# igd-geo/schwarzwald

Measured on AMD Instinct MI355X. Metric: Mpoints/s end-to-end tile (Morton+sort+sample), higher is better.
Workload: dtype u64 keys / f64 positions

## Files before the change

### schwarzwald_amd/csrc/swz_mdblock.hip

```cpp
#include <algorithm>
#include <cmath>
#include <cstdio>
#include <cstdlib>

#include "swz_md.h"
#include "swz_scan.h"

namespace swz {

#ifndef SB_MINW
#define SB_MINW 6
#endif
constexpr int SB_THREADS = 256;
constexpr int SB_K = 4;
constexpr int SB_PEND = 63;
constexpr uint32_t SB_CNT_SAT = 128;
static_assert(SB_CNT_SAT + SB_PEND <= 255u, "a point's neighbour count must not carry into the next point's byte");
static_assert(SB_CNT_SAT > (uint32_t)SB_K, "a saturated count must still read as 'more than the list holds'");
constexpr int SB_PMAX = 12;
constexpr uint32_t SB_NC = 64;
constexpr uint32_t SB_CTR_STRIDE = 32;
constexpr uint32_t SB_NONE = 0xFFFFFFFFu;
enum : uint32_t { SB_U = 0, SB_A = 1, SB_R = 2 };
enum : uint32_t { SB_ABORT_NONE = 0, SB_ABORT_CAPACITY = 1, SB_ABORT_TIMEOUT = 2 };
enum : uint32_t { SBW_ABORT = 0, SBW_MAX_OWN = 1, SBW_MAX_HALO = 2, SBW_ITER = 3, SBW_BLOCKS = 4, SBW_WAITS = 5, SBW_RESEARCH = 6, SBW_STEPS = 7,
                  SBW_T0 = 8 , SBW_COUNT = 16 };
#ifdef SWZ_SB_STATS
#define SB_T(i) do { if (tid == 0) { const uint64_t now_ = wall_clock64(); tacc[i] += (uint32_t)(now_ - tlast); tlast = now_; } } while (0)
#else
#define SB_T(i) do { } while (0)
#endif
enum : uint32_t { SBM_SN = 0, SBM_B = 1, SBM_FIRST = 2, SBM_NOWN = 3, SBM_ABORT = 4, SBM_COUNT = 8 };

struct SbArgs {
  const uint64_t* akey;
  uint32_t m;
  const uint2* gtab;
  uint32_t* st2;
  uint8_t* taken;
  const uint32_t* aidx;
  const uint32_t* perm;
  const double* xyz;
  float f_lo, f_hi;
  uint32_t i_lo, i_hi;
  double sq_spacing;
  uint32_t cell_bits;
  uint32_t cl;
  uint32_t ns;
  uint32_t* ctr;
  uint32_t own_cap, halo_cap;
  uint64_t timeout_ticks;
};

__device__ __forceinline__ uint32_t sb_expand3(uint32_t v) {
  v = (v | (v << 16)) & 0x030000FFu;
  v = (v | (v << 8)) & 0x0300F00Fu;
  v = (v | (v << 4)) & 0x030C30C3u;
  v = (v | (v << 2)) & 0x09249249u;
  return v;
}
__device__ __forceinline__ uint32_t sb_load_word(const uint32_t* p) { return __hip_atomic_load(p, __ATOMIC_RELAXED, __HIP_MEMORY_SCOPE_AGENT); }
__device__ __forceinline__ uint32_t sb_lds_state(const uint8_t* st, uint32_t q) {
  return __hip_atomic_load(st + q, __ATOMIC_RELAXED, __HIP_MEMORY_SCOPE_WORKGROUP);
}
__device__ __forceinline__ void sb_lds_set(uint8_t* st, uint32_t q, uint32_t v) {
  __hip_atomic_store(st + q, (uint8_t)v, __ATOMIC_RELAXED, __HIP_MEMORY_SCOPE_WORKGROUP);
}
__device__ __forceinline__ uint64_t sb_pack(uint32_t x, uint32_t y, uint32_t z) { return (uint64_t)x | ((uint64_t)y << 21) | ((uint64_t)z << 42); }
__device__ __forceinline__ void sb_unpack(uint64_t p, uint32_t& x, uint32_t& y, uint32_t& z) {
  const uint32_t lo = (uint32_t)p, hi = (uint32_t)(p >> 32);
  x = lo & 0x1FFFFFu;
  y = ((lo >> 21) | (hi << 11)) & 0x1FFFFFu;
  z = hi >> 10;
}
constexpr uint32_t SB_CELL_NONE = 0xFFFu;

__device__ __forceinline__ bool sb_exact_near(const SbArgs& a, uint32_t gp, uint32_t gq) {
  const uint32_t sp = a.aidx ? a.aidx[gp] : gp, sq = a.aidx ? a.aidx[gq] : gq;
  const double* u = a.xyz + (size_t)a.perm[sp] * 3;
  const double* v = a.xyz + (size_t)a.perm[sq] * 3;
  return sq_dist(u[0], u[1], u[2], v[0], v[1], v[2]) < a.sq_spacing;
}

struct SbLds {
  uint64_t* pts;
  uint32_t* cse;
  uint32_t* occ;
  uint32_t* soff;
  uint32_t* sfirst;
  uint32_t* pub;
  uint32_t* misc;
  uint32_t* scan;
  uint16_t* nbr;
  uint8_t* st;
  uint32_t* cnt4;
  uint32_t* pend;
};
__host__ __device__ inline size_t sb_lds_bytes(uint32_t own_cap, uint32_t halo_cap) {
  const size_t tot = (size_t)own_cap + halo_cap;
  size_t b = tot * 8;
  b += 1024 * 4 + 128 * 4 + 224 * 4 + 224 * 4;
  b += (((size_t)own_cap / 16 + 5) & ~(size_t)1) * 4 + SBM_COUNT * 4 + 8 * 4;
  b += std::max((size_t)own_cap * SB_K, tot) * 2;
  b += ((tot + 3) & ~(size_t)3) + own_cap + 4 * (SB_PEND + 1) * 4;
  return (b + 15) & ~(size_t)15;
}
__device__ __forceinline__ SbLds sb_carve(unsigned char* smem, uint32_t own_cap, uint32_t halo_cap) {
  const uint32_t tot = own_cap + halo_cap;
  SbLds l;
  l.pts = reinterpret_cast<uint64_t*>(smem);
  l.cse = reinterpret_cast<uint32_t*>(l.pts + tot);
  l.occ = l.cse + 1024;
  l.soff = l.occ + 128;
  l.sfirst = l.soff + 224;
  l.pub = l.sfirst + 224;
  l.misc = l.pub + ((own_cap / 16 + 5u) & ~1u);
  l.scan = l.misc + SBM_COUNT;
  l.nbr = reinterpret_cast<uint16_t*>(l.scan + 8);
  l.st = reinterpret_cast<uint8_t*>(l.nbr + max(own_cap * (uint32_t)SB_K, tot));
  l.cnt4 = reinterpret_cast<uint32_t*>(l.st + ((tot + 3u) & ~3u));
  l.pend = l.cnt4 + own_cap / 4u;
  return l;
}

struct SbBlock {
  uint32_t first;
  uint32_t n_own;
  uint32_t bx8, by8, bz8;
};
__device__ __forceinline__ uint32_t sb_region_cell(const SbArgs& a, const SbBlock& k, uint32_t x, uint32_t y, uint32_t z) {
  const uint32_t cmask = (1u << a.cl) - 1u;
  const uint32_t ix = ((x >> a.cell_bits) & cmask) - k.bx8 + 1u, iy = ((y >> a.cell_bits) & cmask) - k.by8 + 1u, iz = ((z >> a.cell_bits) & cmask) - k.bz8 + 1u;
  return (ix < 10u && iy < 10u && iz < 10u) ? (ix | (iy << 4) | (iz << 8)) : SB_CELL_NONE;
}
__device__ __forceinline__ uint32_t sb_cell_index(uint32_t c) { return (c & 15u) + 10u * ((c >> 4) & 15u) + 100u * (c >> 8); }
template <bool WIDE>
__device__ __forceinline__ uint64_t sb_make_point(const SbArgs& a, const SbBlock& k, uint32_t x, uint32_t y, uint32_t z, uint32_t* cell) {
  const uint32_t c = sb_region_cell(a, k, x, y, z);
  *cell = c;
  if (WIDE) return sb_pack(x, y, z);
  const uint32_t nmask = (1u << (a.cell_bits + a.cl)) - 1u;
  const uint32_t xr = (x & nmask) - ((k.bx8 - 1u) << a.cell_bits), yr = (y & nmask) - ((k.by8 - 1u) << a.cell_bits),
                 zr = (z & nmask) - ((k.bz8 - 1u) << a.cell_bits);
  return (uint64_t)((xr & 0xFFFFu) | (yr << 16)) | ((uint64_t)((zr & 0xFFFFu) | (c << 16)) << 32);
}
__device__ __forceinline__ uint32_t sb_halo_slot(const SbLds& l, uint32_t j) {
  uint32_t lo = 0;
#pragma unroll
  for (uint32_t step = 128u; step; step >>= 1)
    if (lo + step <= 216u && l.soff[lo + step] <= j) lo += step;
  return lo;
}
__device__ __forceinline__ uint32_t sb_active_index(const SbLds& l, const SbBlock& k, uint32_t q) {
  if (q < k.n_own) return k.first + q;
  const uint32_t slot = sb_halo_slot(l, q);
  return l.sfirst[slot] + (q - l.soff[slot]);
}

__device__ __forceinline__ uint32_t sb_earlier_mask(uint32_t ix, uint32_t iy, uint32_t iz) {
  const uint32_t lx = ix - 1u, ly = iy - 1u, lz = iz - 1u;
  const int mx = 3 * (int)__builtin_ctz(lx | 8u) + 2, my = 3 * (int)__builtin_ctz(ly | 8u) + 1, mz = 3 * (int)__builtin_ctz(lz | 8u);
  const int px = 3 * (int)__builtin_ctz(~lx) + 2, py = 3 * (int)__builtin_ctz(~ly) + 1, pz = 3 * (int)__builtin_ctz(~lz);
  uint32_t m = 0x361Bu;
  m |= (mx > py ? 1u : 0u) << 15;
  m |= (my > px ? 1u : 0u) << 11;
  m |= (mx > pz ? 1u : 0u) << 21;
  m |= (mz > px ? 1u : 0u) << 5;
  m |= (my > pz ? 1u : 0u) << 19;
  m |= (mz > py ? 1u : 0u) << 7;
  m |= (max(mx, my) > pz ? 1u : 0u) << 18;
  m |= (max(mx, mz) > py ? 1u : 0u) << 6;
  m |= (max(my, mz) > px ? 1u : 0u) << 2;
  m |= (mx > max(py, pz) ? 1u : 0u) << 24;
  m |= (my > max(px, pz) ? 1u : 0u) << 20;
  m |= (mz > max(px, py) ? 1u : 0u) << 8;
  const uint32_t hx = (ix == 1u ? 1u : 0u) | (ix == 8u ? 4u : 0u);
  const uint32_t hy = (iy == 1u ? 7u : 0u) | (iy == 8u ? 7u << 6 : 0u);
  const uint32_t hz = (iz == 1u ? 0x1FFu : 0u) | (iz == 8u ? 0x1FFu << 18 : 0u);
  return m | hx * 0x1249249u | hy * 0x40201u | hz;
}

struct SbOwn {
  uint32_t ux, uy, uz;
  float fx, fy, fz;
  uint32_t corner;
  uint32_t mask;
};
template <bool WIDE>
__device__ __forceinline__ SbOwn sb_own_point(const SbArgs& a, const SbLds& l, const SbBlock& k, uint32_t j) {
  SbOwn p;
  const uint64_t me = l.pts[j];
  uint32_t cell;
  if (WIDE) {
    sb_unpack(me, p.ux, p.uy, p.uz);
    cell = sb_region_cell(a, k, p.ux, p.uy, p.uz);
  } else {
    const uint32_t lo = (uint32_t)me, hi = (uint32_t)(me >> 32);
    p.ux = lo & 0xFFFFu;
    p.uy = lo >> 16;
    p.uz = hi & 0xFFFFu;
    cell = hi >> 16;
  }
  p.fx = (float)p.ux;
  p.fy = (float)p.uy;
  p.fz = (float)p.uz;
  const uint32_t ix = cell & 15u, iy = (cell >> 4) & 15u, iz = cell >> 8;
  uint32_t mask = 0;
#pragma unroll
  for (int i = 0; i < 9; ++i) {
    const uint32_t row = l.occ[(iz + (uint32_t)(i / 3) - 1u) * 10u + (iy + (uint32_t)(i % 3) - 1u)];
    mask |= ((row >> (ix - 1u)) & 7u) << (3 * i);
  }
  mask &= sb_earlier_mask(ix, iy, iz);
  if (!WIDE && mask) {
    const uint32_t cs = 1u << a.cell_bits;
    const int ox = (int)(p.ux & (cs - 1u)), oy = (int)(p.uy & (cs - 1u)), oz = (int)(p.uz & (cs - 1u));
    const uint32_t gx[3] = {(uint32_t)__mul24(ox, ox), 0u, (uint32_t)__mul24((int)cs - ox, (int)cs - ox)};
    const uint32_t gy[3] = {(uint32_t)__mul24(oy, oy), 0u, (uint32_t)__mul24((int)cs - oy, (int)cs - oy)};
    const uint32_t gz[3] = {(uint32_t)__mul24(oz, oz), 0u, (uint32_t)__mul24((int)cs - oz, (int)cs - oz)};
    uint32_t reach = 0;
#pragma unroll 1
    for (int zi = 0; zi < 3; ++zi) {
      const uint32_t gzz = zi == 0 ? gz[0] : (zi == 1 ? 0u : gz[2]);
      uint32_t r9 = 0;
#pragma unroll
      for (int b = 0; b < 9; ++b)
        if (gx[b % 3] + gy[b / 3] + gzz < a.i_hi) r9 |= 1u << b;
      reach |= r9 << (9 * zi);
    }
    mask &= reach;
  }
  p.mask = mask;
  p.corner = (ix - 1u) + 10u * (iy - 1u) + 100u * (iz - 1u);
  return p;
}
template <bool WIDE>
__device__ __forceinline__ void sb_compare(const SbArgs& a, const SbOwn& p, uint64_t o, bool& sure, bool& maybe) {
  if (WIDE) {
    uint32_t vx, vy, vz;
    sb_unpack(o, vx, vy, vz);
    const float ddx = p.fx - (float)vx, ddy = p.fy - (float)vy, ddz = p.fz - (float)vz;
    const float d2 = ddx * ddx + ddy * ddy + ddz * ddz;
    sure = d2 < a.f_lo;
    maybe = d2 < a.f_hi;
  } else {
    const uint32_t lo = (uint32_t)o, hi = (uint32_t)(o >> 32);
    const int ddx = (int)p.ux - (int)(lo & 0xFFFFu), ddy = (int)p.uy - (int)(lo >> 16), ddz = (int)p.uz - (int)(hi & 0xFFFFu);
    const uint32_t d2 = (uint32_t)(__mul24(ddx, ddx) + __mul24(ddy, ddy) + __mul24(ddz, ddz));
    sure = d2 < a.i_lo;
    maybe = d2 < a.i_hi;
  }
}
__device__ __forceinline__ uint32_t sb_cell_offset(uint32_t b) {
  const uint32_t dz = (b * 57u) >> 9, rem = b - 9u * dz, dy = (rem * 11u) >> 5, dx = rem - 3u * dy;
  return dx + 10u * dy + 100u * dz;
}

template <bool WIDE, typename F>
__device__ __forceinline__ void sb_visit(const SbArgs& a, const SbLds& l, const SbBlock& k, uint32_t j, F f) {
  const SbOwn p = sb_own_point<WIDE>(a, l, k, j);
  uint32_t mask = p.mask;
  uint32_t q = 0, e = 0;
  for (;;) {
    if (q >= e) {
      if (!mask) break;
      const uint32_t b = (uint32_t)__ffs((int)mask) - 1u;
      mask &= mask - 1u;
      const uint32_t e2 = l.cse[p.corner + sb_cell_offset(b)];
      q = e2 & 0xFFFFu;
      e = e2 >> 16;
      if (q < k.n_own) e = min(e, j);
      if (q >= e) continue;
    }
    bool sure, maybe;
    sb_compare<WIDE>(a, p, l.pts[q], sure, maybe);
    if (maybe) {
      if (sure || sb_exact_near(a, k.first + j, sb_active_index(l, k, q))) {
        if (!f(q)) return;
      }
    }
    ++q;
  }
}

template <bool WIDE>
__device__ __forceinline__ void sb_search(const SbArgs& a, const SbLds& l, const SbBlock& k, uint32_t j, bool active, uint16_t* mine,
                                          uint32_t* pend, uint32_t* cnt_out, uint32_t* steps) {
  const SbOwn p = sb_own_point<WIDE>(a, l, k, active ? j : 0u);
  uint32_t mask = active ? p.mask : 0u;
  uint32_t q = 0, e = 0, cnt = 0;
  uint32_t ne2 = l.cse[mask ? p.corner + sb_cell_offset((uint32_t)__ffs((int)mask) - 1u) : 0u];
  while (__ballot(active)) {
    ++*steps;
    const bool need = active && q >= e;
    const bool fetch = need && mask != 0u;
    const uint32_t s2 = ne2 & 0xFFFFu, t2 = ne2 >> 16;
    const uint32_t t3 = s2 < k.n_own ? min(t2, j) : t2;
    mask = fetch ? (mask & (mask - 1u)) : mask;
    q = fetch ? s2 : q;
    e = fetch ? t3 : e;
    active = active && !(need && !fetch);
    if (__ballot(fetch)) {
      const uint32_t nxt = l.cse[(fetch && mask) ? p.corner + sb_cell_offset((uint32_t)__ffs((int)mask) - 1u) : 0u];
      ne2 = fetch ? nxt : ne2;
    }
    const bool valid = active && q < e;
    bool sure, maybe;
    sb_compare<WIDE>(a, p, l.pts[valid ? q : 0u], sure, maybe);
    maybe = maybe && valid;
    if (__ballot(maybe)) {
      const bool band = maybe && !sure;
      bool near = maybe && sure;
      if (__ballot(band)) {
        if (band) {
          const uint32_t slot = atomicAdd(&pend[SB_PEND], 1u);
          if (slot < (uint32_t)SB_PEND) pend[slot] = (j << 16) | q;
          else near = sb_exact_near(a, k.first + j, sb_active_index(l, k, q));
        }
      }
      if (near && cnt < (uint32_t)SB_K) mine[cnt] = (uint16_t)q;
      cnt += near ? 1u : 0u;
    }
    q += valid ? 1u : 0u;
  }
  *cnt_out = cnt;
}

__device__ __forceinline__ uint32_t sb_state_of(const SbArgs& a, const SbLds& l, const SbBlock& k, uint32_t q, bool poll) {
  uint32_t s = sb_lds_state(l.st, q);
  if (poll && s == SB_U && q >= k.n_own) {
    const uint32_t gi = sb_active_index(l, k, q);
    s = (sb_load_word(a.st2 + (gi >> 4)) >> ((gi & 15u) * 2u)) & 3u;
    if (s != SB_U) sb_lds_set(l.st, q, s);
  }
  return s;
}

template <bool WIDE>
__global__ __launch_bounds__(SB_THREADS, SB_MINW) void sb_block_kernel(SbArgs a) {
  extern __shared__ __align__(16) unsigned char sb_smem[];
  const SbLds l = sb_carve(sb_smem, a.own_cap, a.halo_cap);
  const uint32_t tid = threadIdx.x, lane = tid & 63u, wave = tid >> 6;
  const uint32_t nb_per_node = 1u << (3u * (a.cl - 3u));
  const uint32_t gmax = 1u << (a.cl - 1u);
  const uint64_t gran_per_node = 1ull << (3u * (a.cl - 1u));
  uint32_t* words = a.ctr + SB_NC * SB_CTR_STRIDE;
  uint32_t kc = (blockIdx.x & 7u) + 8u * ((blockIdx.x >> 3) % (SB_NC / 8u));
  uint32_t tried = 0;
  uint32_t my_blocks = 0, my_iters = 0, my_waits = 0, my_research = 0, my_steps = 0;
  uint16_t* rc = l.nbr;
#ifdef SWZ_SB_STATS
  uint32_t tacc[8] = {0, 0, 0, 0, 0, 0, 0, 0};
  uint64_t tlast = wall_clock64();
#endif
  if (tid == 0) l.misc[SBM_ABORT] = 0;

  for (;;) {
    if (tid == 0) {
      uint32_t sn = SB_NONE, b = 0;
      if (l.misc[SBM_ABORT] == 0 && sb_load_word(words + SBW_ABORT) == SB_ABORT_NONE) {
        while (tried < SB_NC) {
          const uint32_t nodes_k = a.ns > kc ? (a.ns - kc + SB_NC - 1u) / SB_NC : 0u;
          if (nodes_k) {
            const uint32_t t = __hip_atomic_fetch_add(a.ctr + kc * SB_CTR_STRIDE, 1u, __ATOMIC_RELAXED, __HIP_MEMORY_SCOPE_AGENT);
            if ((uint64_t)t < (uint64_t)nodes_k * nb_per_node) {
              sn = (t % nodes_k) * SB_NC + kc;
              b = t / nodes_k;
              break;
            }
          }
          kc = (kc + 1u) % SB_NC;
          ++tried;
        }
      }
      l.misc[SBM_SN] = sn;
      l.misc[SBM_B] = b;
      l.misc[SBM_FIRST] = SB_NONE;
      l.misc[SBM_NOWN] = 0;
    }
    if (tid < 128u) l.occ[tid] = 0u;
    __syncthreads();
    SB_T(0);
    const uint32_t sn = l.misc[SBM_SN], b = l.misc[SBM_B];
    if (sn == SB_NONE) break;

    const uint32_t bx = contract_bits_by_3_u32(b >> 2), by = contract_bits_by_3_u32(b >> 1), bz = contract_bits_by_3_u32(b);
    const uint2* gt = a.gtab + (uint64_t)sn * gran_per_node;
    uint32_t own_cnt = 0, halo_cnt = 0, run_first = 0;
    if (tid < 216u) {
      const uint32_t rx = tid % 6u, ry = (tid / 6u) % 6u, rz = tid / 36u;
      const int gx = (int)(bx * 4u + rx) - 1, gy = (int)(by * 4u + ry) - 1, gz = (int)(bz * 4u + rz) - 1;
      const bool inner = rx - 1u < 4u && ry - 1u < 4u && rz - 1u < 4u;
      if (gx >= 0 && gy >= 0 && gz >= 0 && gx < (int)gmax && gy < (int)gmax && gz < (int)gmax) {
        const uint32_t code = (sb_expand3((uint32_t)gx) << 2) | (sb_expand3((uint32_t)gy) << 1) | sb_expand3((uint32_t)gz);
        if (inner || code < (b << 6)) {
          const uint2 e = gt[code];
          if (e.y) {
            run_first = e.x;
            if (inner) own_cnt = e.y - e.x; else halo_cnt = e.y - e.x;
          }
        }
      }
      if (own_cnt) {
        atomicMin(&l.misc[SBM_FIRST], run_first);
        atomicAdd(&l.misc[SBM_NOWN], own_cnt);
      }
      l.sfirst[tid] = run_first;
    }
    uint32_t n_halo = 0;
    const uint32_t halo_off = block_excl_sum<SB_THREADS>(min(halo_cnt, 0xFFFFFu), l.scan, n_halo);
    SbBlock k;
    k.n_own = l.misc[SBM_NOWN];
    k.first = l.misc[SBM_FIRST];
    k.bx8 = bx * 8u;
    k.by8 = by * 8u;
    k.bz8 = bz * 8u;
    const uint32_t n_own = k.n_own;
    if (n_own == 0) {
      __syncthreads();
      continue;
    }
    const uint32_t total = n_own + n_halo;
    if (n_own > a.own_cap || n_halo > a.halo_cap) {
      if (tid == 0) {
        __hip_atomic_fetch_max(words + SBW_MAX_OWN, n_own, __ATOMIC_RELAXED, __HIP_MEMORY_SCOPE_AGENT);
        __hip_atomic_fetch_max(words + SBW_MAX_HALO, n_halo, __ATOMIC_RELAXED, __HIP_MEMORY_SCOPE_AGENT);
        __hip_atomic_fetch_max(words + SBW_ABORT, (uint32_t)SB_ABORT_CAPACITY, __ATOMIC_RELAXED, __HIP_MEMORY_SCOPE_AGENT);
      }
      break;
    }
    if (tid < 216u) l.soff[tid] = n_own + halo_off;
    if (tid == 216u) l.soff[216] = total;
    const uint32_t w0 = k.first >> 4;
    const uint32_t nw = ((k.first + n_own - 1u) >> 4) - w0 + 1u;
    for (uint32_t w = tid; w < nw; w += SB_THREADS) l.pub[w] = 0u;
    __syncthreads();
    SB_T(1);

#pragma unroll 1
    for (uint32_t half = 0; half < (uint32_t)SB_PMAX; half += 3u) {
      if (half * SB_THREADS >= total) break;
      uint32_t gi[3];
#pragma unroll
      for (int p = 0; p < 3; ++p) {
        const uint32_t j = tid + (half + (uint32_t)p) * SB_THREADS;
        gi[p] = SB_NONE;
        if (j < n_own) {
          gi[p] = k.first + j;
        } else if (j < total) {
          const uint32_t lo = sb_halo_slot(l, j);
          gi[p] = l.sfirst[lo] + (j - l.soff[lo]);
        }
      }
      uint64_t key[3];
      uint32_t sw[3];
#pragma unroll
      for (int p = 0; p < 3; ++p) {
        const uint32_t j = tid + (half + (uint32_t)p) * SB_THREADS;
        key[p] = 0;
        sw[p] = 0;
        if (gi[p] != SB_NONE) {
          key[p] = a.akey[gi[p]];
          if (j >= n_own) sw[p] = sb_load_word(a.st2 + (gi[p] >> 4));
        }
      }
#pragma unroll
      for (int p = 0; p < 3; ++p) {
        const uint32_t j = tid + (half + (uint32_t)p) * SB_THREADS;
        if (gi[p] == SB_NONE) continue;
        uint32_t x, y, z, cell;
        key_coords_u32(key[p], x, y, z);
        l.pts[j] = sb_make_point<WIDE>(a, k, x, y, z, &cell);
        rc[j] = (uint16_t)cell;
        l.st[j] = (uint8_t)((sw[p] >> ((gi[p] & 15u) * 2u)) & 3u);
      }
    }
    __syncthreads();
    SB_T(2);
    for (uint32_t j = tid; j < total; j += SB_THREADS) {
      const uint32_t r = rc[j];
      if (r == SB_CELL_NONE) continue;
      uint16_t* e = reinterpret_cast<uint16_t*>(l.cse + sb_cell_index(r));
      if (j == 0 || rc[j - 1] != r) {
        e[0] = (uint16_t)j;
        atomicOr(&l.occ[(r >> 8) * 10u + ((r >> 4) & 15u)], 1u << (r & 15u));
      }
      if (j + 1 == total || rc[j + 1] != r) e[1] = (uint16_t)(j + 1);
    }
    __syncthreads();
    SB_T(3);

    const uint32_t wa = wave * nw / 4u, wb = (wave + 1u) * nw / 4u;
    const uint32_t ja = max(k.first, (w0 + wa) << 4) - k.first;
    const uint32_t jb = wa < wb ? min(k.first + n_own, (w0 + wb) << 4) - k.first : ja;
    uint32_t* pend = l.pend + wave * (uint32_t)(SB_PEND + 1);
    uint8_t* cnt1 = reinterpret_cast<uint8_t*>(l.cnt4);
    if (lane == 0) pend[SB_PEND] = 0u;
    for (uint32_t base = ja; base < jb; base += 64u) {
      const uint32_t j = base + lane;
      const bool have = j < jb;
      uint32_t cnt = 0;
      sb_search<WIDE>(a, l, k, j, have, l.nbr + (size_t)(have ? j : 0u) * SB_K, pend, &cnt, &my_steps);
      if (have) cnt1[j] = (uint8_t)min(cnt, SB_CNT_SAT);
    }
    {
      const uint32_t np = min(pend[SB_PEND], (uint32_t)SB_PEND);
      for (uint32_t i = lane; i < np; i += 64u) {
        const uint32_t j = pend[i] >> 16, q = pend[i] & 0xFFFFu;
        if (!sb_exact_near(a, k.first + j, sb_active_index(l, k, q))) continue;
        const uint32_t slot = (atomicAdd(&l.cnt4[j >> 2], 1u << (8u * (j & 3u))) >> (8u * (j & 3u))) & 0xFFu;
        if (slot < (uint32_t)SB_K) l.nbr[(size_t)j * SB_K + slot] = (uint16_t)q;
      }
    }
    for (uint32_t base = ja; base < jb; base += 64u) {
      const uint32_t j = base + lane;
      if (j >= jb) continue;
      const uint32_t cnt = cnt1[j];
      uint32_t dec = SB_U;
      if (cnt == 0u) {
        dec = SB_A;
      } else {
        static_assert(SB_K == 4, "four two-byte entries = one eight-byte load");
        uint64_t* slot = reinterpret_cast<uint64_t*>(l.nbr + (size_t)j * SB_K);
        const uint64_t n4 = *slot;
        const uint32_t c4 = min(cnt, (uint32_t)SB_K);
        uint32_t st[SB_K];
#pragma unroll
        for (int i = 0; i < SB_K; ++i) st[i] = (uint32_t)i < c4 ? sb_lds_state(l.st, (uint32_t)(n4 >> (16 * i)) & 0xFFFFu) : (uint32_t)SB_R;
        uint64_t kept = 0;
        uint32_t nk = 0;
        bool any_a = false;
#pragma unroll
        for (int i = 0; i < SB_K; ++i) {
          any_a |= st[i] == SB_A;
          if (st[i] == SB_U) {
            kept |= ((n4 >> (16 * i)) & 0xFFFFull) << (16u * nk);
            ++nk;
          }
        }
        if (any_a) {
          dec = SB_R;
        } else if (cnt <= (uint32_t)SB_K) {
          if (nk == 0u) {
            dec = SB_A;
          } else if (nk != cnt) {
            *slot = kept;
            cnt1[j] = (uint8_t)nk;
          }
        }
      }
      if (dec != SB_U) {
        sb_lds_set(l.st, j, dec);
        const uint32_t gi = k.first + j;
        atomicOr(&l.pub[(gi >> 4) - w0], dec << ((gi & 15u) * 2u));
      }
    }
    SB_T(4);
    uint64_t t_idle = 0;
    uint32_t idle = 0;
    bool gave_up = false, poll = false, to_publish = true;
    for (;;) {
      bool remaining = false, progress = false, halo_wait = false;
      for (uint32_t base = ja; base < jb; base += 64u) {
        const uint32_t j = base + lane;
        const bool have = j < jb;
        uint32_t cur = have ? sb_lds_state(l.st, j) : (uint32_t)SB_R;
        const bool und = have && cur == SB_U;
        if (!__ballot(und)) continue;
        static_assert(SB_K == 4, "four two-byte entries = one eight-byte load");
        const uint32_t cnt = und ? cnt1[j] : 0u;
        const uint64_t n4 = und ? *reinterpret_cast<const uint64_t*>(l.nbr + (size_t)j * SB_K) : 0ull;
        const uint32_t c4 = min(cnt, (uint32_t)SB_K);
        uint32_t q[SB_K], st[SB_K];
        uint32_t inround = 0;
#pragma unroll
        for (int i = 0; i < SB_K; ++i) {
          q[i] = (uint32_t)(n4 >> (16 * i)) & 0xFFFFu;
          const bool used = (uint32_t)i < c4;
          const bool here = used && q[i] >= base && q[i] < min(base + 64u, jb);
          inround |= here ? 1u << i : 0u;
          st[i] = used && !here ? sb_lds_state(l.st, q[i]) : (uint32_t)SB_R;
        }
        bool ext_a = false, ext_u = false;
#pragma unroll
        for (int i = 0; i < SB_K; ++i) {
          uint32_t v = st[i];
          if (poll && v == SB_U && q[i] >= k.n_own) v = sb_state_of(a, l, k, q[i], true);
          ext_a |= v == SB_A;
          ext_u |= v == SB_U;
          halo_wait |= v == SB_U && q[i] >= k.n_own;
        }
        const bool listed = und && cnt <= (uint32_t)SB_K;
        bool in_u_last = false;
        for (;;) {
          bool in_a = false, in_u = false;
#pragma unroll
          for (int i = 0; i < SB_K; ++i) {
            const uint32_t sv = (uint32_t)__shfl((int)cur, (int)((q[i] - base) & 63u), WAVE);
            if ((inround >> i) & 1u) {
              in_a |= sv == SB_A;
              in_u |= sv == SB_U;
            }
          }
          in_u_last = in_u;
          bool changed = false;
          if (und && cur == SB_U) {
            if (ext_a || in_a) {
              cur = SB_R;
              changed = true;
            } else if (listed && !ext_u && !in_u) {
              cur = SB_A;
              changed = true;
            }
          }
          if (!__ballot(changed)) break;
        }
        if (und && cur == SB_U && cnt > (uint32_t)SB_K && !ext_u && !in_u_last) {
          bool any_a = false, any_u = false;
          ++my_research;
          sb_visit<WIDE>(a, l, k, j, [&](uint32_t qq) {
            const uint32_t sv = sb_state_of(a, l, k, qq, true);
            any_a |= sv == SB_A;
            any_u |= sv == SB_U;
            return !any_a;
          });
          if (any_a) cur = SB_R; else if (!any_u) cur = SB_A;
        }
        if (und && cur != SB_U) {
          sb_lds_set(l.st, j, cur);
          const uint32_t gi = k.first + j;
          atomicOr(&l.pub[(gi >> 4) - w0], cur << ((gi & 15u) * 2u));
          progress = true;
        } else if (und) {
          remaining = true;
        }
      }
      const bool any_progress = __ballot(progress) != 0, any_remaining = __ballot(remaining) != 0;
      if (lane == 0) ++my_iters;
      to_publish |= any_progress;
      if (any_progress && any_remaining && !poll) continue;
      if (to_publish) {
        for (uint32_t w = wa + lane; w < wb; w += 64u) {
          const uint32_t v = atomicExch(&l.pub[w], 0u);
          if (v) __hip_atomic_fetch_or(a.st2 + w0 + w, v, __ATOMIC_RELAXED, __HIP_MEMORY_SCOPE_AGENT);
        }
        to_publish = false;
      }
      if (!any_remaining) break;
      if (any_progress) {
        idle = 0;
        t_idle = 0;
        poll = false;
        continue;
      }
      poll = __ballot(halo_wait) != 0;
      ++idle;
      if (lane == 0) ++my_waits;
      if (idle > 1u) __builtin_amdgcn_s_sleep(4);
      if ((idle & 15u) == 0u) {
        uint32_t stop = 0;
        if (lane == 0) {
          const uint64_t now = wall_clock64();
          if (t_idle == 0) t_idle = now;
          if (sb_load_word(words + SBW_ABORT) != SB_ABORT_NONE || __hip_atomic_load(&l.misc[SBM_ABORT], __ATOMIC_RELAXED, __HIP_MEMORY_SCOPE_WORKGROUP)) {
            stop = 1;
          } else if (now - t_idle > a.timeout_ticks) {
            __hip_atomic_fetch_max(words + SBW_ABORT, (uint32_t)SB_ABORT_TIMEOUT, __ATOMIC_RELAXED, __HIP_MEMORY_SCOPE_AGENT);
            stop = 1;
          }
        }
        if (__shfl((int)stop, 0, WAVE)) {
          gave_up = true;
          break;
        }
      }
    }
    SB_T(5);
    if (gave_up) {
      if (lane == 0) __hip_atomic_store(&l.misc[SBM_ABORT], 1u, __ATOMIC_RELAXED, __HIP_MEMORY_SCOPE_WORKGROUP);
    } else {
      for (uint32_t base = ja; base < jb; base += 64u) {
        const uint32_t j = base + lane;
        if (j < jb && sb_lds_state(l.st, j) == SB_A) a.taken[k.first + j] = 1;
      }
    }
    if (tid == 0) ++my_blocks;
    __syncthreads();
    SB_T(6);
  }
#ifdef SWZ_SB_STATS
  if (tid == 0)
    for (int i = 0; i < 7; ++i) atomicAdd(words + SBW_T0 + i, tacc[i] >> 4);
#endif
  if (lane == 0) {
    if (my_blocks) atomicAdd(words + SBW_BLOCKS, my_blocks);
    if (my_iters) atomicAdd(words + SBW_ITER, my_iters);
    if (my_waits) atomicAdd(words + SBW_WAITS, my_waits);
    if (my_steps) atomicAdd(words + SBW_STEPS, my_steps);
  }
  if (my_research) atomicAdd(words + SBW_RESEARCH, my_research);
}

struct SbTabArgs {
  const uint64_t* akey;
  const uint32_t* nid;
  const uint8_t* nmode;
  const uint32_t* snode_of;
  const uint32_t* sn_direct;
  uint32_t all_sampled;
  uint32_t m;
  uint32_t gran_shift;
  uint64_t gran_per_node;
  uint2* gtab;
};
__device__ __forceinline__ uint64_t sb_granule_of(const SbTabArgs& t, uint32_t i) {
  uint32_t sn;
  if (t.sn_direct) {
    sn = t.sn_direct[i];
  } else {
    const uint32_t node = t.nid[i];
    if (!t.all_sampled && t.nmode[node] != MODE_SAMPLE) return ~0ull;
    sn = t.all_sampled ? node : t.snode_of[node];
  }
  return (uint64_t)sn * t.gran_per_node + ((t.akey[i] >> t.gran_shift) & (t.gran_per_node - 1ull));
}
__global__ __launch_bounds__(256) void sb_table_kernel(SbTabArgs t) {
  const uint32_t i = blockIdx.x * 256 + threadIdx.x;
  if (i >= t.m) return;
  const uint64_t g = sb_granule_of(t, i);
  if (g == ~0ull) return;
  const bool head = i == 0 || sb_granule_of(t, i - 1) != g;
  const bool tail = i + 1 == t.m || sb_granule_of(t, i + 1) != g;
  if (head) t.gtab[g].x = i;
  if (tail) t.gtab[g].y = i + 1u;
}

struct SbInput {
  const uint64_t* akey = nullptr;
  uint32_t m = 0;
  const uint32_t* aidx = nullptr;
  const uint32_t* sn_direct = nullptr;
  uint8_t* taken = nullptr;
  uint32_t points = 0;
  const uint32_t* occupied = nullptr;
  double spread = 1.0;
  const char* what = "";
};

static int sb_run(swz_ctx* c, const MdLevel& L, const SbInput& in, bool* done) {
  *done = false;
  const LevelPlan& plan = L.plan;
  const SortedPoints& sp = L.sp;
  const LevelBuffers& lb = L.lb;
  const KeyMetric& km = L.km;
  const uint32_t sample_nodes = L.sample_nodes;
  const bool dbg = c->opt("SWZ_DEBUG") != nullptr;
  int cl = plan.cell_levels_geo;
  const double min_block = c->opt_num("SWZ_SP_BLOCK_MIN", 128.0);
  auto per_block = [&](int l) { return (double)in.points / (double)std::max(1u, in.occupied[std::max(0, l - 3)]); };
  while (cl > 3 && per_block(cl) < min_block) --cl;
  bool cl_forced = false, caps_forced = false;
  if (const char* e = c->opt("SWZ_SP_BLOCK_CL")) {
    cl = std::min(plan.cell_levels_geo, atoi(e));
    cl_forced = true;
  }
  if (cl < 3 || cl > 10) return SWZ_OK;
  const uint32_t limit = (uint32_t)(SB_THREADS * SB_PMAX);
  auto estimate = [&](int l, uint32_t* own, uint32_t* halo) {
    const double expect = per_block(l), dev = std::sqrt(expect * in.spread);
    *own = (uint32_t)std::max(128.0, 32.0 * std::ceil((expect + (in.spread > 2.0 ? 6.0 : 8.0) * dev + 32.0) / 32.0));
    *halo = (uint32_t)(32.0 * std::ceil((1.25 * expect + (in.spread > 2.0 ? 7.0 : 10.0) * std::sqrt(1.25) * dev + 64.0) / 32.0));
  };
  auto fill_free_lds = [&](uint32_t* own, uint32_t* halo) {
    const size_t free_lds = 26u * 1024u;
    const uint32_t own_max = *own + *own / 2u, halo_max = *halo + *halo / 2u;
    for (bool grew = true; grew;) {
      grew = false;
      if (*halo + 32u <= halo_max && *own + *halo + 32u <= limit && sb_lds_bytes(*own, *halo + 32u) <= free_lds) *halo += 32u, grew = true;
      if (*own + 32u <= own_max && *own + 32u < limit / 2u && *own + *halo + 32u <= limit && sb_lds_bytes(*own + 32u, *halo) <= free_lds)
        *own += 32u, grew = true;
    }
  };
  uint32_t own_cap = 0, halo_cap = 0;
  estimate(cl, &own_cap, &halo_cap);
  fill_free_lds(&own_cap, &halo_cap);
  const double cap_scale = c->opt_num("SWZ_SP_BLOCK_CAP_SCALE", 1.0);
  if (cap_scale != 1.0) {
    own_cap = std::max(32u, (uint32_t)(own_cap * cap_scale) / 32u * 32u);
    halo_cap = std::max(32u, (uint32_t)(halo_cap * cap_scale) / 32u * 32u);
  }
  if (const char* e = c->opt("SWZ_SP_BLOCK_OWN")) {
    own_cap = (uint32_t)std::max(64, atoi(e)) / 16u * 16u;
    caps_forced = true;
  }
  if (const char* e = c->opt("SWZ_SP_BLOCK_HALO")) {
    halo_cap = (uint32_t)std::max(64, atoi(e)) / 16u * 16u;
    caps_forced = true;
  }
  const uint32_t node_shift = plan.node_shift;
  SbTabArgs t{};
  t.akey = in.akey;
  t.nid = lb.nid;
  t.nmode = lb.nmode;
  t.snode_of = L.snode_of;
  t.sn_direct = in.sn_direct;
  t.all_sampled = L.all_sampled ? 1u : 0u;
  t.m = in.m;
  SbArgs a{};
  a.akey = in.akey;
  a.m = in.m;
  SWZ_TRY(c->get("sb_state", (size_t)in.m / 16 + 2, &a.st2));
  a.taken = in.taken;
  a.aidx = in.aidx;
  a.perm = sp.perm;
  a.xyz = sp.xyz;
  a.f_lo = km.f_lo;
  a.f_hi = km.f_hi;
  if (c->opt_num("SWZ_SP_FILTER_EPS", 0.0) >= 0.5) {
    a.f_lo = 0.f;
    a.f_hi = INFINITY;
  }
  a.i_lo = a.f_lo >= 4294967040.f ? 0xFFFFFFFFu : (uint32_t)std::floor(a.f_lo);
  a.i_hi = a.f_hi >= 4294967040.f ? 0xFFFFFFFFu : (uint32_t)std::ceil(a.f_hi);
  a.sq_spacing = plan.sq_spacing;
  a.ns = sample_nodes;
  SWZ_TRY(c->get("sb_counters", (size_t)(SB_NC * SB_CTR_STRIDE + SBW_COUNT), &a.ctr));
  const double timeout_s = c->opt_num("SWZ_SP_BLOCK_TIMEOUT_MS", 10000.0) * 1e-3;
  a.timeout_ticks = (uint64_t)(timeout_s * 1e8);
  int cus = 256;
  (void)hipDeviceGetAttribute(&cus, hipDeviceAttributeMultiprocessorCount, c->device);

  for (int attempt = 0; attempt < 4; ++attempt) {
    if (own_cap + halo_cap > limit) {
      if (own_cap >= limit / 2u) return SWZ_OK;
      halo_cap = limit - own_cap;
    }
    const size_t lds = sb_lds_bytes(own_cap, halo_cap);
    if (lds > 160u * 1024u) return SWZ_OK;
    const uint64_t gran_per_node = 1ull << (3 * (cl - 1));
    const uint64_t entries = (uint64_t)sample_nodes * gran_per_node;
    if (entries > (1ull << 30)) return SWZ_OK;
    t.gran_shift = node_shift - 3u * (uint32_t)(cl - 1);
    t.gran_per_node = gran_per_node;
    SWZ_TRY(c->get("sb_gtab", (size_t)entries, &t.gtab));
    a.gtab = t.gtab;
    a.cell_bits = (node_shift - 3u * (uint32_t)cl) / 3u;
    a.cl = (uint32_t)cl;
    a.own_cap = own_cap;
    a.halo_cap = halo_cap;

    ProfScope ps(c, "sample_min_distance", attempt == 0 ? (uint64_t)in.points * 33ull : 0ull, 1);
    SWZ_HIP(c, memset_large(t.gtab, 0, (size_t)entries * sizeof(uint2), c->stream));
    SWZ_HIP(c, hipMemsetAsync(a.st2, 0, ((size_t)in.m / 16 + 2) * sizeof(uint32_t), c->stream));
    SWZ_HIP(c, hipMemsetAsync(a.ctr, 0, (size_t)(SB_NC * SB_CTR_STRIDE + SBW_COUNT) * sizeof(uint32_t), c->stream));
    hipLaunchKernelGGL(sb_table_kernel, dim3(div_up(in.m, 256)), dim3(256), 0, c->stream, t);
    SWZ_LAUNCH_CHECK(c);
    const bool wide = a.cell_bits > 12u || c->opt_on("SWZ_SP_BLOCK_WIDE", false);
    SWZ_HIP(c, hipFuncSetAttribute(reinterpret_cast<const void*>(wide ? sb_block_kernel<true> : sb_block_kernel<false>),
                                   hipFuncAttributeMaxDynamicSharedMemorySize, 160 * 1024));
    uint32_t per_cu = (uint32_t)std::max<size_t>(1, std::min<size_t>(8, (160u * 1024u) / lds));
    per_cu = (uint32_t)std::max(1L, c->opt_int("SWZ_SP_BLOCK_PER_CU", per_cu));
    const uint64_t blocks_total = (uint64_t)sample_nodes << (3 * (cl - 3));
    const uint32_t grid = (uint32_t)std::min<uint64_t>((uint64_t)cus * per_cu, std::max<uint64_t>(1, blocks_total));
    hipEvent_t ev0 = nullptr, ev1 = nullptr;
    if (dbg) {
      ev0 = c->take_event();
      ev1 = c->take_event();
      (void)hipEventRecord(ev0, c->stream);
    }
    if (wide)
      hipLaunchKernelGGL(sb_block_kernel<true>, dim3(grid), dim3(SB_THREADS), lds, c->stream, a);
    else
      hipLaunchKernelGGL(sb_block_kernel<false>, dim3(grid), dim3(SB_THREADS), lds, c->stream, a);
    SWZ_LAUNCH_CHECK(c);
    if (dbg) (void)hipEventRecord(ev1, c->stream);
    uint32_t h[SBW_COUNT] = {0};
    SWZ_HIP(c, hipMemcpyAsync(h, a.ctr + SB_NC * SB_CTR_STRIDE, sizeof(h), hipMemcpyDeviceToHost, c->stream));
    SWZ_HIP(c, hipStreamSynchronize(c->stream));
    if (dbg) {
      float ms = 0.f;
      (void)hipEventElapsedTime(&ms, ev0, ev1);
      c->event_pool.insert(c->event_pool.end(), {ev0, ev1});
      fprintf(stderr,
              "[swz] MIN_DISTANCE level %d block path%s: %u pts in %u nodes, cell_levels %d (geo %d), %.0f pts/block, caps %u / %u, LDS %zu B, "
              "grid %u, %u blocks, %u search steps, %u passes, %u idle passes, %u searched again, abort %u (max %u / %u), %.2f ms\n",
              plan.level, in.what, in.points, sample_nodes, cl, plan.cell_levels_geo, per_block(cl), own_cap, halo_cap, lds, grid, h[SBW_BLOCKS],
              h[SBW_STEPS], h[SBW_ITER], h[SBW_WAITS], h[SBW_RESEARCH], h[SBW_ABORT], h[SBW_MAX_OWN], h[SBW_MAX_HALO], ms);
    }
#ifdef SWZ_SB_STATS
    if (dbg && h[SBW_BLOCKS])
      fprintf(stderr, "[swz]   thread 0, us per block: ticket %.2f, granules %.2f, stage %.2f, index %.2f, search %.2f, decide %.2f, tail %.2f\n",
              h[SBW_T0] * 0.16 / h[SBW_BLOCKS], h[SBW_T0 + 1] * 0.16 / h[SBW_BLOCKS], h[SBW_T0 + 2] * 0.16 / h[SBW_BLOCKS], h[SBW_T0 + 3] * 0.16 / h[SBW_BLOCKS],
              h[SBW_T0 + 4] * 0.16 / h[SBW_BLOCKS], h[SBW_T0 + 5] * 0.16 / h[SBW_BLOCKS], h[SBW_T0 + 6] * 0.16 / h[SBW_BLOCKS]);
#endif
    if (h[SBW_ABORT] == SB_ABORT_TIMEOUT)
      return c->fail(SWZ_ERR_INTERNAL, "MIN_DISTANCE block path: a workgroup waited longer than the time-out for an earlier block");
    if (h[SBW_ABORT] == SB_ABORT_NONE) {
      *done = true;
      return SWZ_OK;
    }
    if (caps_forced) return SWZ_OK;
    const uint32_t need_own = std::max(own_cap, (h[SBW_MAX_OWN] + h[SBW_MAX_OWN] / 4u + 63u) / 32u * 32u);
    const uint32_t need_halo = std::max(halo_cap, (h[SBW_MAX_HALO] + h[SBW_MAX_HALO] / 4u + 95u) / 32u * 32u);
    if (need_own < limit / 2u && need_own + need_halo <= limit) {
      own_cap = need_own;
      halo_cap = need_halo;
    } else if (cl < plan.cell_levels_geo && !cl_forced && per_block(cl + 1) >= 0.5 * min_block) {
      ++cl;
      estimate(cl, &own_cap, &halo_cap);
      fill_free_lds(&own_cap, &halo_cap);
    } else {
      return SWZ_OK;
    }
  }
  return SWZ_OK;
}

struct SbiArgs {
  const uint64_t* akey;
  const uint32_t* aidx;
  const uint32_t* nid;
  const uint8_t* nmode;
  const uint32_t* snode_of;
  const uint8_t* indep;
  uint32_t all_sampled;
  uint32_t m;
  uint32_t old_lo, old_n;
  uint32_t cell_shift;
  uint32_t cell_mask;
  uint32_t cl;
  uint32_t* bits;
  uint8_t* sel;
  uint8_t* taken;
};
__global__ __launch_bounds__(256) void sbi_indep_kernel(const uint32_t* __restrict__ nstart, const uint8_t* __restrict__ nmode,
                                                        uint32_t nnodes, const uint64_t* __restrict__ akey, uint32_t nsh,
                                                        const uint64_t* __restrict__ ckey, uint32_t nc, uint64_t max_points,
                                                        const uint64_t* __restrict__ child_nkey, uint32_t child_nn,
                                                        uint8_t* __restrict__ indep) {
  const uint32_t j = blockIdx.x * 256 + threadIdx.x;
  if (j >= nnodes) return;
  uint8_t r = 0;
  if (nmode[j] == MODE_SAMPLE) {
    const uint64_t prefix = akey[nstart[j]] >> nsh;
    uint32_t lo = 0, hi = nc;
    while (lo < hi) {
      const uint32_t mid = lo + (hi - lo) / 2;
      if ((ckey[mid] >> nsh) < prefix) lo = mid + 1; else hi = mid;
    }
    const uint32_t first = lo;
    hi = nc;
    while (lo < hi) {
      const uint32_t mid = lo + (hi - lo) / 2;
      if ((ckey[mid] >> nsh) <= prefix) lo = mid + 1; else hi = mid;
    }
    const uint32_t cached = lo - first;
    r = (uint64_t)cached > max_points ? 1 : 0;
    if (!r && cached && child_nn) {
      const uint64_t from = prefix << nsh;
      lo = 0;
      hi = child_nn;
      while (lo < hi) {
        const uint32_t mid = lo + (hi - lo) / 2;
        if (child_nkey[mid] < from) lo = mid + 1; else hi = mid;
      }
      r = lo < child_nn && (child_nkey[lo] >> nsh) == prefix ? 1 : 0;
    }
  }
  indep[j] = r;
}
__device__ __forceinline__ bool sbi_sampled(const SbiArgs& a, uint32_t i, uint32_t* node) {
  *node = a.nid[i];
  return a.all_sampled || a.nmode[*node] == MODE_SAMPLE;
}
__device__ __forceinline__ bool sbi_is_old(const SbiArgs& a, uint32_t i, uint32_t node) {
  return a.aidx[i] - a.old_lo < a.old_n && a.indep[node];
}
__device__ __forceinline__ uint64_t sbi_cell_base(const SbiArgs& a, uint32_t node) {
  return (uint64_t)(a.all_sampled ? node : a.snode_of[node]) << (3u * a.cl);
}
template <bool CLEAR>
__global__ __launch_bounds__(256) void sbi_mark_kernel(SbiArgs a, const uint64_t* __restrict__ new_key, uint32_t new_m,
                                                       const uint32_t* __restrict__ nstart, uint32_t nnodes, uint32_t nsh) {
  const uint32_t i = blockIdx.x * 256 + threadIdx.x;
  if (i >= new_m) return;
  const uint64_t key = new_key[i], prefix = key >> nsh;
  uint32_t lo = 0, hi = nnodes;
  while (lo < hi) {
    const uint32_t mid = lo + (hi - lo) / 2u;
    if ((a.akey[nstart[mid]] >> nsh) <= prefix) lo = mid + 1u; else hi = mid;
  }
  if (lo == 0) return;
  const uint32_t node = lo - 1u;
  if ((a.akey[nstart[node]] >> nsh) != prefix || !(a.all_sampled || a.nmode[node] == MODE_SAMPLE) || !a.indep[node]) return;
  const uint64_t bit = sbi_cell_base(a, node) + ((uint32_t)(key >> a.cell_shift) & a.cell_mask);
  const uint32_t b = 1u << (uint32_t)(bit & 31ull);
  uint32_t* w = a.bits + (bit >> 5);
  if (CLEAR) {
    *w = 0u;
  } else if (!(__hip_atomic_load(w, __ATOMIC_RELAXED, __HIP_MEMORY_SCOPE_AGENT) & b)) {
    atomicOr(w, b);
  }
}
__device__ __forceinline__ bool sbi_near_new(const SbiArgs& a, uint64_t base, uint32_t code) {
  const uint32_t gmask = a.cell_mask >> 3;
  const uint32_t MX = 0x09249249u & gmask, MY = 0x12492492u & gmask, MZ = 0x24924924u & gmask;
  const uint32_t g = code >> 3, x = g & MX, y = g & MY, z = g & MZ;
  const uint8_t* marks = reinterpret_cast<const uint8_t*>(a.bits) + (base >> 3);
// ... 226 lines not shown
```

Baseline: 2487.

## Streamline neighbour search branching and vectorise granule table kernel

Makes the warp-level search loop branch-free: the explicit active flag is dropped, the next cell entry is always fetched through a sentinel-safe index, and the maybe test folds validity into its threshold. The cell-offset computation becomes a single packed mul24, the halo binary search becomes branchless, and the wave index is made scalar via readfirstlane. The granule table kernel now handles four keys per thread with vector loads and compares key prefixes before looking up node ids, skipping those lookups for interior points. The unconditional LDS load of the next entry adds work when no fetch is needed, and the head/tail test assumes equal key prefixes imply the same sample node.

```diff
diff --git a/schwarzwald_amd/csrc/swz_mdblock.hip b/schwarzwald_amd/csrc/swz_mdblock.hip
--- a/schwarzwald_amd/csrc/swz_mdblock.hip
+++ b/schwarzwald_amd/csrc/swz_mdblock.hip
@@ -59,6 +59,7 @@
   v = (v | (v << 2)) & 0x09249249u;
   return v;
 }
+__device__ __forceinline__ bool sb_any(bool p) { return __builtin_amdgcn_ballot_w64(p) != 0ull; }
 __device__ __forceinline__ uint32_t sb_load_word(const uint32_t* p) { return __hip_atomic_load(p, __ATOMIC_RELAXED, __HIP_MEMORY_SCOPE_AGENT); }
 __device__ __forceinline__ uint32_t sb_lds_state(const uint8_t* st, uint32_t q) {
   return __hip_atomic_load(st + q, __ATOMIC_RELAXED, __HIP_MEMORY_SCOPE_WORKGROUP);
@@ -147,8 +148,10 @@
 __device__ __forceinline__ uint32_t sb_halo_slot(const SbLds& l, uint32_t j) {
   uint32_t lo = 0;
 #pragma unroll
-  for (uint32_t step = 128u; step; step >>= 1)
-    if (lo + step <= 216u && l.soff[lo + step] <= j) lo += step;
+  for (uint32_t step = 128u; step; step >>= 1) {
+    const uint32_t probe = min(lo + step, 216u);
+    lo += l.soff[probe] <= j ? step : 0u;
+  }
   return lo;
 }
 __device__ __forceinline__ uint32_t sb_active_index(const SbLds& l, const SbBlock& k, uint32_t q) {
@@ -235,25 +238,28 @@
   return p;
 }
 template <bool WIDE>
-__device__ __forceinline__ void sb_compare(const SbArgs& a, const SbOwn& p, uint64_t o, bool& sure, bool& maybe) {
+__device__ __forceinline__ void sb_compare(const SbArgs& a, const SbOwn& p, uint64_t o, bool valid, bool& sure, bool& maybe) {
   if (WIDE) {
     uint32_t vx, vy, vz;
     sb_unpack(o, vx, vy, vz);
     const float ddx = p.fx - (float)vx, ddy = p.fy - (float)vy, ddz = p.fz - (float)vz;
     const float d2 = ddx * ddx + ddy * ddy + ddz * ddz;
     sure = d2 < a.f_lo;
-    maybe = d2 < a.f_hi;
+    maybe = d2 < (valid ? a.f_hi : 0.f);
   } else {
     const uint32_t lo = (uint32_t)o, hi = (uint32_t)(o >> 32);
     const int ddx = (int)p.ux - (int)(lo & 0xFFFFu), ddy = (int)p.uy - (int)(lo >> 16), ddz = (int)p.uz - (int)(hi & 0xFFFFu);
     const uint32_t d2 = (uint32_t)(__mul24(ddx, ddx) + __mul24(ddy, ddy) + __mul24(ddz, ddz));
     sure = d2 < a.i_lo;
-    maybe = d2 < a.i_hi;
+    maybe = d2 < (valid ? a.i_hi : 0u);
   }
 }
 __device__ __forceinline__ uint32_t sb_cell_offset(uint32_t b) {
-  const uint32_t dz = (b * 57u) >> 9, rem = b - 9u * dz, dy = (rem * 11u) >> 5, dx = rem - 3u * dy;
-  return dx + 10u * dy + 100u * dz;
+  const uint32_t x = (uint32_t)__mul24((int)b, (int)((57u << 16) | 11u));
+  return b + 7u * ((x >> 5) & 15u) + 70u * (x >> 25);
+}
+__device__ __forceinline__ uint32_t sb_next_entry(uint32_t corner, uint32_t mask) {
+  return corner + sb_cell_offset((uint32_t)__builtin_ctz(mask | (1u << 26)));
 }
 
 template <bool WIDE, typename F>
@@ -273,7 +279,7 @@
       if (q >= e) continue;
     }
     bool sure, maybe;
-    sb_compare<WIDE>(a, p, l.pts[q], sure, maybe);
+    sb_compare<WIDE>(a, p, l.pts[q], true, sure, maybe);
     if (maybe) {
       if (sure || sb_exact_near(a, k.first + j, sb_active_index(l, k, q))) {
         if (!f(q)) return;
@@ -284,34 +290,29 @@
 }
 
 template <bool WIDE>
-__device__ __forceinline__ void sb_search(const SbArgs& a, const SbLds& l, const SbBlock& k, uint32_t j, bool active, uint16_t* mine,
+__device__ __forceinline__ void sb_search(const SbArgs& a, const SbLds& l, const SbBlock& k, uint32_t j, bool have, uint16_t* mine,
                                           uint32_t* pend, uint32_t* cnt_out, uint32_t* steps) {
-  const SbOwn p = sb_own_point<WIDE>(a, l, k, active ? j : 0u);
-  uint32_t mask = active ? p.mask : 0u;
+  const SbOwn p = sb_own_point<WIDE>(a, l, k, have ? j : 0u);
+  uint32_t mask = have ? p.mask : 0u;
   uint32_t q = 0, e = 0, cnt = 0;
-  uint32_t ne2 = l.cse[mask ? p.corner + sb_cell_offset((uint32_t)__ffs((int)mask) - 1u) : 0u];
-  while (__ballot(active)) {
+  uint32_t ne2 = l.cse[sb_next_entry(p.corner, mask)];
+  while ((__builtin_amdgcn_ballot_w64(q < e) | __builtin_amdgcn_ballot_w64(mask != 0u)) != 0ull) {
     ++*steps;
-    const bool need = active && q >= e;
-    const bool fetch = need && mask != 0u;
+    const bool fetch = q >= e && mask != 0u;
     const uint32_t s2 = ne2 & 0xFFFFu, t2 = ne2 >> 16;
     const uint32_t t3 = s2 < k.n_own ? min(t2, j) : t2;
     mask = fetch ? (mask & (mask - 1u)) : mask;
     q = fetch ? s2 : q;
     e = fetch ? t3 : e;
-    active = active && !(need && !fetch);
-    if (__ballot(fetch)) {
-      const uint32_t nxt = l.cse[(fetch && mask) ? p.corner + sb_cell_offset((uint32_t)__ffs((int)mask) - 1u) : 0u];
-      ne2 = fetch ? nxt : ne2;
-    }
-    const bool valid = active && q < e;
+    const uint32_t nxt = l.cse[sb_next_entry(p.corner, mask)];
+    ne2 = fetch ? nxt : ne2;
+    const bool valid = q < e;
     bool sure, maybe;
-    sb_compare<WIDE>(a, p, l.pts[valid ? q : 0u], sure, maybe);
-    maybe = maybe && valid;
-    if (__ballot(maybe)) {
+    sb_compare<WIDE>(a, p, l.pts[valid ? q : 0u], valid, sure, maybe);
+    if (sb_any(maybe)) {
       const bool band = maybe && !sure;
       bool near = maybe && sure;
-      if (__ballot(band)) {
+      if (sb_any(band)) {
         if (band) {
           const uint32_t slot = atomicAdd(&pend[SB_PEND], 1u);
           if (slot < (uint32_t)SB_PEND) pend[slot] = (j << 16) | q;
@@ -340,7 +341,8 @@
 __global__ __launch_bounds__(SB_THREADS, SB_MINW) void sb_block_kernel(SbArgs a) {
   extern __shared__ __align__(16) unsigned char sb_smem[];
   const SbLds l = sb_carve(sb_smem, a.own_cap, a.halo_cap);
-  const uint32_t tid = threadIdx.x, lane = tid & 63u, wave = tid >> 6;
+  const uint32_t tid = threadIdx.x, lane = tid & 63u;
+  const uint32_t wave = (uint32_t)__builtin_amdgcn_readfirstlane((int)(tid >> 6));
   const uint32_t nb_per_node = 1u << (3u * (a.cl - 3u));
   const uint32_t gmax = 1u << (a.cl - 1u);
   const uint64_t gran_per_node = 1ull << (3u * (a.cl - 1u));
@@ -566,7 +568,7 @@
         const bool have = j < jb;
         uint32_t cur = have ? sb_lds_state(l.st, j) : (uint32_t)SB_R;
         const bool und = have && cur == SB_U;
-        if (!__ballot(und)) continue;
+        if (!sb_any(und)) continue;
         static_assert(SB_K == 4, "four two-byte entries = one eight-byte load");
         const uint32_t cnt = und ? cnt1[j] : 0u;
         const uint64_t n4 = und ? *reinterpret_cast<const uint64_t*>(l.nbr + (size_t)j * SB_K) : 0ull;
@@ -613,7 +615,7 @@
               changed = true;
             }
           }
-          if (!__ballot(changed)) break;
+          if (!sb_any(changed)) break;
         }
         if (und && cur == SB_U && cnt > (uint32_t)SB_K && !ext_u && !in_u_last) {
           bool any_a = false, any_u = false;
@@ -635,7 +637,7 @@
           remaining = true;
         }
       }
-      const bool any_progress = __ballot(progress) != 0, any_remaining = __ballot(remaining) != 0;
+      const bool any_progress = sb_any(progress), any_remaining = sb_any(remaining);
       if (lane == 0) ++my_iters;
       to_publish |= any_progress;
       if (any_progress && any_remaining && !poll) continue;
@@ -653,7 +655,7 @@
         poll = false;
         continue;
       }
-      poll = __ballot(halo_wait) != 0;
+      poll = sb_any(halo_wait);
       ++idle;
       if (lane == 0) ++my_waits;
       if (idle > 1u) __builtin_amdgcn_s_sleep(4);
@@ -713,26 +715,40 @@
   uint64_t gran_per_node;
   uint2* gtab;
 };
-__device__ __forceinline__ uint64_t sb_granule_of(const SbTabArgs& t, uint32_t i) {
-  uint32_t sn;
-  if (t.sn_direct) {
-    sn = t.sn_direct[i];
+__global__ __launch_bounds__(256) void sb_table_kernel(SbTabArgs t, uint32_t vec) {
+  const uint64_t i0 = ((uint64_t)blockIdx.x * 256u + threadIdx.x) * 4u;
+  if (i0 >= t.m) return;
+  const uint32_t n = t.m - i0 < 4u ? (uint32_t)(t.m - i0) : 4u;
+  uint64_t key[6];
+  if (vec && n == 4u) {
+    const ulonglong2 v0 = *reinterpret_cast<const ulonglong2*>(t.akey + i0), v1 = *reinterpret_cast<const ulonglong2*>(t.akey + i0 + 2);
+    key[1] = v0.x, key[2] = v0.y, key[3] = v1.x, key[4] = v1.y;
   } else {
-    const uint32_t node = t.nid[i];
-    if (!t.all_sampled && t.nmode[node] != MODE_SAMPLE) return ~0ull;
-    sn = t.all_sampled ? node : t.snode_of[node];
-  }
-  return (uint64_t)sn * t.gran_per_node + ((t.akey[i] >> t.gran_shift) & (t.gran_per_node - 1ull));
-}
-__global__ __launch_bounds__(256) void sb_table_kernel(SbTabArgs t) {
-  const uint32_t i = blockIdx.x * 256 + threadIdx.x;
-  if (i >= t.m) return;
-  const uint64_t g = sb_granule_of(t, i);
-  if (g == ~0ull) return;
-  const bool head = i == 0 || sb_granule_of(t, i - 1) != g;
-  const bool tail = i + 1 == t.m || sb_granule_of(t, i + 1) != g;
-  if (head) t.gtab[g].x = i;
-  if (tail) t.gtab[g].y = i + 1u;
+#pragma unroll
+    for (uint32_t j = 0; j < 4u; ++j) key[1 + j] = j < n ? t.akey[i0 + j] : 0ull;
+  }
+  key[0] = i0 ? t.akey[i0 - 1u] : 0ull;
+  key[5] = i0 + 4u < t.m ? t.akey[i0 + 4u] : 0ull;
+#pragma unroll
+  for (uint32_t j = 0; j < 4u; ++j) {
+    if (j >= n) break;
+    const uint32_t i = (uint32_t)i0 + j;
+    const uint64_t pre = key[1 + j] >> t.gran_shift;
+    const bool head = i == 0u || (key[j] >> t.gran_shift) != pre;
+    const bool tail = i + 1u == t.m || (key[2 + j] >> t.gran_shift) != pre;
+    if (!head && !tail) continue;
+    uint32_t sn;
+    if (t.sn_direct) {
+      sn = t.sn_direct[i];
+    } else {
+      const uint32_t node = t.nid[i];
+      if (!t.all_sampled && t.nmode[node] != MODE_SAMPLE) continue;
+      sn = t.all_sampled ? node : t.snode_of[node];
+    }
+    const uint64_t g = (uint64_t)sn * t.gran_per_node + (pre & (t.gran_per_node - 1ull));
+    if (head) t.gtab[g].x = i;
+    if (tail) t.gtab[g].y = i + 1u;
+  }
 }
 
 struct SbInput {
@@ -853,7 +869,7 @@
     SWZ_HIP(c, memset_large(t.gtab, 0, (size_t)entries * sizeof(uint2), c->stream));
     SWZ_HIP(c, hipMemsetAsync(a.st2, 0, ((size_t)in.m / 16 + 2) * sizeof(uint32_t), c->stream));
     SWZ_HIP(c, hipMemsetAsync(a.ctr, 0, (size_t)(SB_NC * SB_CTR_STRIDE + SBW_COUNT) * sizeof(uint32_t), c->stream));
-    hipLaunchKernelGGL(sb_table_kernel, dim3(div_up(in.m, 256)), dim3(256), 0, c->stream, t);
+    hipLaunchKernelGGL(sb_table_kernel, dim3(div_up(in.m, 1024)), dim3(256), 0, c->stream, t, ((uintptr_t)t.akey & 15u) == 0 ? 1u : 0u);
     SWZ_LAUNCH_CHECK(c);
     const bool wide = a.cell_bits > 12u || c->opt_on("SWZ_SP_BLOCK_WIDE", false);
     SWZ_HIP(c, hipFuncSetAttribute(reinterpret_cast<const void*>(wide ? sb_block_kernel<true> : sb_block_kernel<false>),
```

Result: faster. 2549, median of 6 (+2.5%).
